# openai/baselines

Measured on NVIDIA H100. Metric: PPO2 learner env-steps/sec, higher is better.
Workload: dtype f16 operands / f32 accumulate (GAE f64 carry)

## Files before the change

baselines_b200/csrc/conv_shift.cu:

```cuda
#include <stdlib.h>

#include <type_traits>

#include "common.cuh"
#include "tc_common.cuh"

namespace b200rl {

static constexpr int SH_BM = 128;
static constexpr int SH_CONSUMER_WARPS = 8;
static constexpr int SH_TMA_WARP = SH_CONSUMER_WARPS;
__host__ __device__ constexpr int sh_threads(bool u8) { return (SH_CONSUMER_WARPS + 1) * 32 + (u8 ? 256 : 0); }
static constexpr int SH_MAX_TAPS = 16;
__host__ __device__ constexpr int sh_arows(int KH) { return KH == 1 ? 160 : 144; }
__host__ __device__ constexpr int sh_stages(int KH) { return KH == 1 ? 6 : 4; }
static constexpr int SH_U8_STAGES = 12;
static constexpr int SH_U8_WRES_BYTES = 16 * 1024;
__host__ __device__ constexpr int sh_wgrad_krows(bool u8) { return u8 ? 128 : 64; }
__host__ __device__ constexpr int sh_wres_bytes(int KH, bool u8) {
  return u8 ? SH_U8_WRES_BYTES : KH == 1 ? 80 * 1024 : 64 * 1024;
}
static constexpr int SH_BAR_BYTES = 512;
__host__ __device__ constexpr int sh_mask_stage_bytes(int BN, bool DACT) { return DACT ? SH_BM * BN / 8 : 0; }
static constexpr int SH_EPI_WARP_BYTES = 16 * 64;
static constexpr int SH_EPI_BYTES = SH_CONSUMER_WARPS * SH_EPI_WARP_BYTES;
static constexpr int SH_WROWS_K = 96;
static constexpr int SH_WABYTES = SH_WROWS_K * 128;
__host__ __device__ constexpr int sh_wgrad_qw(int BN, int KH, bool u8) { return u8 ? 2 : BN == 32 ? 4 : KH == 1 ? 3 : 2; }

static constexpr int SH_ORDER_BAR = 2;
__device__ __forceinline__ void order_wait(int wg) {
  asm volatile("bar.sync %0, %1;" ::"r"(SH_ORDER_BAR + wg), "n"(SH_CONSUMER_WARPS * 32) : "memory");
}
__device__ __forceinline__ void order_pass(int wg) {
  asm volatile("bar.arrive %0, %1;" ::"r"(SH_ORDER_BAR + 1 - wg), "n"(SH_CONSUMER_WARPS * 32) : "memory");
}

struct AddrMap {
  int mode;
  long long sN, sY, sX;
  int Cq, s;
  int Cq_log2, s_log2;
};

__device__ __forceinline__ long long map_rowbase(const AddrMap& a, int n, int y, int x) {
  if (a.mode == 2) {
    const int sm = a.s - 1;
// ... 137 lines not shown
          }
        }
        fence_proxy_async_smem();
        __syncwarp();
        if (lane == 0) {
          if (tile < ntiles) mbar_arrive(&full_bar[s]);
          if (ub == 0) mbar_arrive(&head_bar[s]);
        }
        u8_load(u, row_start, uc + RND, sb[d], lane, q[d]);
        sb[d] = u8_lookup(u, row_start, uc + 2 * RND, total, M, lane);
      }
    }
  }
}

struct ShiftParams {
  U8Src u8;
  FastDiv fwg, fhg;
  long long M;
  int Hg, Wg;
  int N;
  int taps;
  int shift[SH_MAX_TAPS];
  int min_shift;
  int vy, vx;
  __half* out;
  AddrMap omap;
  uint16_t* bits_out;
  const uint16_t* saved_bits;
  const float* bias;
  int act, dact;
  float alpha;
  int num_tiles;
};

__device__ __forceinline__ void stmatrix_x4(uint32_t addr, const uint32_t (&r)[4]) {
  asm volatile("stmatrix.sync.aligned.m8n8.x4.shared.b16 [%0], {%1, %2, %3, %4};" ::"r"(addr), "r"(r[0]), "r"(r[1]),
               "r"(r[2]), "r"(r[3])
               : "memory");
}
__device__ __forceinline__ uint4 ld_shared_v4(uint32_t addr) {
  uint4 v;
  asm volatile("ld.shared.v4.b32 {%0,%1,%2,%3}, [%4];" : "=r"(v.x), "=r"(v.y), "=r"(v.z), "=r"(v.w) : "r"(addr) : "memory");
  return v;
}
__device__ __forceinline__ void st_global_v4(void* p, const uint4& v) {
  asm volatile("st.global.v4.b32 [%0], {%1,%2,%3,%4};" ::"l"(p), "r"(v.x), "r"(v.y), "r"(v.z), "r"(v.w) : "memory");
}
__device__ __forceinline__ uint32_t h2_bits(__half2 h) { return *reinterpret_cast<const uint32_t*>(&h); }
__device__ __forceinline__ uint32_t mask_pair(uint32_t b8, int k) {
  const uint32_t b = b8 >> (2 * k);
  return ((b & 1u) | ((b & 2u) << 15)) * 0xffffu;
}

template <int BN, int KH, bool DACT, bool U8>
__global__ void __launch_bounds__(sh_threads(U8), 1)
conv_shift_fwd_kernel(const __grid_constant__ CUtensorMap tmX, const __grid_constant__ CUtensorMap tmW,
                      const __grid_constant__ ShiftParams p) {
  constexpr int SH_ABYTES = sh_arows(KH) * 128;
  constexpr int STAGE_BYTES = KH * SH_ABYTES;
  constexpr int STAGES = U8 ? SH_U8_STAGES : sh_stages(KH);
  using Ring = U8Ring<SH_BM, STAGES>;
  constexpr bool PINGPONG = !(BN == 128 && !DACT);
  constexpr int MH = PINGPONG ? 2 : 1;
  static_assert(PINGPONG || !U8, "the uint8 ring's release rule assumes ping-pong");
  constexpr int A_PITCH = U8 ? SH_BM * 128 : STAGE_BYTES;
  constexpr int A_TOTAL = U8 ? Ring::BYTES : STAGES * STAGE_BYTES;
  extern __shared__ uint8_t smem_raw[];
  uint8_t* smem = reinterpret_cast<uint8_t*>((reinterpret_cast<uintptr_t>(smem_raw) + 1023) & ~uintptr_t(1023));
  uint8_t* wres = smem + A_TOTAL;
  uint64_t* bars = reinterpret_cast<uint64_t*>(wres + sh_wres_bytes(KH, U8));
  uint64_t* full_bar = bars;
  uint64_t* empty_bar = bars + STAGES;
  uint64_t* w_bar = bars + 2 * STAGES;
  uint64_t* head_bar = bars + 2 * STAGES + 1;
  static_assert((3 * STAGES + 1) * 8 <= SH_BAR_BYTES, "barrier block");
  constexpr int MASK_STAGE = sh_mask_stage_bytes(BN, DACT);
  uint8_t* smask = reinterpret_cast<uint8_t*>(bars) + SH_BAR_BYTES;
  uint8_t* sepi = smask + STAGES * MASK_STAGE;

  __shared__ float s_bias[BN];
  const int warp = threadIdx.x >> 5, lane = threadIdx.x & 31;
  constexpr int w_sub = BN * 128;
  if (threadIdx.x < BN) s_bias[threadIdx.x] = (p.bias && (int)threadIdx.x < p.N) ? p.bias[threadIdx.x] : 0.0f;
  if (threadIdx.x == 0) {
    for (int s = 0; s < STAGES; ++s) {
      mbar_init(&full_bar[s], U8 ? Ring::UPT : 1);
      mbar_init(&empty_bar[s], (U8 || !PINGPONG) ? SH_CONSUMER_WARPS : 4);
      if (U8) mbar_init(&head_bar[s], 1);
    }
    mbar_init(w_bar, 1);
    if (U8)
// ... 11 lines not shown
  } else {
    tile_first = (int)blockIdx.x;
    tile_stride = (int)gridDim.x;
    tile_count = tile_first < p.num_tiles ? (p.num_tiles - tile_first + tile_stride - 1) / tile_stride : 0;
  }

  if (warp == SH_TMA_WARP) {
    if (elect_one()) {
      tma_prefetch_desc(&tmX);
      tma_prefetch_desc(&tmW);
      mbar_arrive_expect_tx(w_bar, (uint32_t)(p.taps * KH) * w_sub);
      for (int q = 0; q < p.taps * KH; ++q) tma_load_2d(wres + q * w_sub, &tmW, w_bar, q * 64, 0);
    }
    __syncwarp();
    int s = 0;
    uint32_t ph = 0;
    if (!U8) {
      for (int i = 0; i < tile_count; ++i) {
        const int tile = tile_first + i * tile_stride;
        mbar_wait(&empty_bar[s], ph ^ 1);
        if (elect_one()) {
          uint8_t* sa = smem + s * STAGE_BYTES;
          uint32_t mbytes = 0;
          const uint8_t* msrc = nullptr;
          if (DACT && p.saved_bits != nullptr) {
            const long long left = p.M - (long long)tile * SH_BM;
            mbytes = (uint32_t)(left < SH_BM ? left : SH_BM) * (BN / 8);
            msrc = reinterpret_cast<const uint8_t*>(p.saved_bits) + (long long)tile * MASK_STAGE;
#pragma unroll 1
            for (uint32_t b = mbytes & ~15u; b < mbytes; b += 4)
              *reinterpret_cast<uint32_t*>(smask + s * MASK_STAGE + b) = __ldg(reinterpret_cast<const uint32_t*>(msrc + b));
            if (mbytes & 15u) __threadfence_block();
          }
          mbar_arrive_expect_tx(&full_bar[s], (uint32_t)STAGE_BYTES + (mbytes & ~15u));
          const int row0 = tile * SH_BM + p.min_shift;
#pragma unroll
          for (int h = 0; h < KH; ++h) tma_load_2d(sa + h * SH_ABYTES, &tmX, &full_bar[s], h * 64, row0);
          if (mbytes >= 16) bulk_load_1d(smask + s * MASK_STAGE, msrc, mbytes & ~15u, &full_bar[s]);
        }
        __syncwarp();
        if (++s == STAGES) { s = 0; ph ^= 1; }
      }
    }
  } else if (U8 && warp > SH_TMA_WARP) {
    u8_ring_producer<SH_BM, STAGES, 2>(p.u8, p.M, (long long)tile_first * SH_BM + p.min_shift, tile_count, smem,
                                       full_bar, head_bar, empty_bar, warp - (SH_TMA_WARP + 1), lane);
  } else {
    const int wg = __shfl_sync(0xffffffffu, warp >> 2, 0), t = threadIdx.x & 127;
    const int row0 = PINGPONG ? 0 : wg * 64;
    const uint32_t w_base = smem_u32(wres);
    const float lo = (p.act == ACT_RELU) ? 0.0f : -INFINITY;
    const __half2 lo2 = __floats2half2_rn(lo, lo);
    const __half2 zero2 = __floats2half2_rn(0.0f, 0.0f);
    const int er = lane & 15, ep = lane >> 4;
    const int erow = row0 + 16 * (warp & 3) + er;
    uint32_t epi_addr[2];
#pragma unroll
    for (int jj = 0; jj < 2; ++jj)
      epi_addr[jj] = smem_u32(sepi + warp * SH_EPI_WARP_BYTES) + er * 64 + (((2 * jj + ep) ^ ((er >> 1) & 3)) << 4);
    const bool masked = DACT && p.saved_bits != nullptr;
    float acc[MH][BN / 2];
    mbar_wait(w_bar, 0);
    for (int i = PINGPONG ? wg : 0; i < tile_count; i += PINGPONG ? 2 : 1) {
      const int tile = tile_first + i * tile_stride;
      const int s = i % STAGES, s1 = (s + 1 == STAGES) ? 0 : s + 1;
      const uint32_t ph = (uint32_t)(i / STAGES) & 1u;
      mbar_wait(&full_bar[s], ph);
      if (U8) mbar_wait(&head_bar[s1], s1 == 0 ? ph ^ 1 : ph);
      if (PINGPONG && i > 0) order_wait(wg);
      const uint32_t a_base = smem_u32(smem + s * A_PITCH) + (uint32_t)(row0 * 128);
      wgmma_fence();
#pragma unroll 1
      for (int a = 0; a < p.taps; ++a) {
        const uint32_t at = a_base + (uint32_t)p.shift[a] * 128u;
        const uint32_t wt = w_base + (uint32_t)(a * KH * w_sub);
#pragma unroll
        for (int h = 0; h < KH; ++h) {
#pragma unroll
          for (int k = 0; k < 4; ++k) {
            const uint64_t bdesc = make_sdesc(wt + h * w_sub + k * 32, 16, 1024, 1);
#pragma unroll
            for (int mh = 0; mh < MH; ++mh) {
              const uint64_t adesc = make_sdesc(at + mh * 64 * 128 + h * SH_ABYTES + k * 32, 16, 1024, 1);
              wgmma_f16<BN, 0, 0>(acc[mh], adesc, bdesc, (a | h | k) ? 1u : 0u);
            }
          }
        }
      }
      wgmma_commit();
      if (PINGPONG && i + 1 < tile_count) order_pass(wg);
      wgmma_wait<0>();
      auto release = [&]() {
        __syncwarp();
        if (lane == 0) {
          mbar_arrive(&empty_bar[s]);
          if (U8) mbar_arrive(&empty_bar[s1]);
        }
      };
      uint32_t mrow[MH][BN / 32];
      if (masked) {
#pragma unroll
        for (int mh = 0; mh < MH; ++mh) {
          const uint32_t r = smem_u32(smask + s * MASK_STAGE) + (uint32_t)((erow + mh * 64) * (BN / 8));
#pragma unroll
          for (int i = 0; i < BN / 32; ++i) asm volatile("ld.shared.b32 %0, [%1];" : "=r"(mrow[mh][i]) : "r"(r + 4 * i));
        }
      } else {
        release();
      }

#pragma unroll
      for (int mh = 0; mh < MH; ++mh) {
        const uint32_t m = (uint32_t)tile * SH_BM + mh * 64 + erow;
        const uint32_t t2 = p.fwg.div(m);
        const int x = (int)(m - t2 * (uint32_t)p.Wg);
        const int n = (int)p.fhg.div(t2);
        const int y = (int)(t2 - (uint32_t)n * (uint32_t)p.Hg);
        const bool ok = ((long long)m < p.M) && (y < p.vy) && (x < p.vx);
        const long long obase = map_rowbase(p.omap, n, y, x);
#pragma unroll
        for (int ps = 0; ps < BN / 32; ++ps) {
#pragma unroll
          for (int jj = 0; jj < 2; ++jj) {
            const int b = 2 * (2 * ps + jj);
            uint32_t r[4];
#pragma unroll
            for (int k = 0; k < 4; ++k) {
              const int e = 4 * (b + (k >> 1)) + 2 * (k & 1);
              const int c = 8 * (b + (k >> 1)) + 2 * (t & 3);
              __half2 o;
              if (DACT) {
                o = __floats2half2_rn(acc[mh][e] * p.alpha, acc[mh][e + 1] * p.alpha);
              } else {
                o = __hmax2(__floats2half2_rn(fmaf(acc[mh][e], p.alpha, s_bias[c]),
                                              fmaf(acc[mh][e + 1], p.alpha, s_bias[c + 1])),
                            lo2);
              }
              r[k] = h2_bits(o);
            }
            stmatrix_x4(epi_addr[jj], r);
          }
          __syncwarp();
#pragma unroll
          for (int jj = 0; jj < 2; ++jj) {
            const int j = 2 * ps + jj;
            uint4 v = ld_shared_v4(epi_addr[jj]);
            const long long ocol = map_coloff(p.omap, 16 * j);
            if (masked) {
              const uint32_t b8 = (mrow[mh][j >> 1] >> (16 * (j & 1) + 8 * ep)) & 0xffu;
              v.x &= mask_pair(b8, 0);
              v.y &= mask_pair(b8, 1);
// ... 224 lines not shown
      }
    }
    if (kb1 > kb0) {
#pragma unroll
      for (int i = 0; i < QW; ++i) {
        if (i < nq) {
#pragma unroll
          for (int e = 0; e < BN / 2; ++e) {
            const int cn = acc_col(t, e);
            const long long grow = (long long)(q0 + i) * 64 + acc_row(t, e);
            if (cn < p.N) p.ws_g[((long long)blockIdx.x * p.grows + grow) * p.N + cn] = acc[i][e] * p.alpha;
          }
        }
      }
    }
  }
  if (ncta > 1) cluster_sync();
}

static U8Src make_u8src(const void* x, const long long* idx, int H, int W, int C, int s) {
  U8Src u{};
  u.x = reinterpret_cast<const uint8_t*>(x);
  if (!x) return u;
  u.idx = idx;
  u.sample_bytes = (long long)H * W * C;
  u.row_bytes = W * C;
  u.y_bytes = s * W * C;
  u.x_bytes = s * C;
  u.per = make_fastdiv((uint32_t)((H / s) * (W / s)));
  u.wg = make_fastdiv((uint32_t)(W / s));
  return u;
}

template <int BN, int KH, bool DACT, bool U8 = false>
static int launch_fwd(const CUtensorMap& tmX, const CUtensorMap& tmW, const ShiftParams& p, cudaStream_t st) {
  constexpr int STAGES = U8 ? SH_U8_STAGES : sh_stages(KH);
  constexpr int SMEM = (U8 ? U8Ring<SH_BM, STAGES>::BYTES : STAGES * KH * sh_arows(KH) * 128) + sh_wres_bytes(KH, U8) +
                       1024 + SH_BAR_BYTES + STAGES * sh_mask_stage_bytes(BN, DACT) + SH_EPI_BYTES;
  static_assert(SMEM + 1024 <= 227 * 1024, "conv_shift_fwd: shared memory budget (+ static bias array)");
  static bool attr = false;
  auto kern = conv_shift_fwd_kernel<BN, KH, DACT, U8>;
  if (!attr) {
    cudaError_t e = cudaFuncSetAttribute(kern, cudaFuncAttributeMaxDynamicSharedMemorySize, SMEM);
    if (e != cudaSuccess) {
      set_last_error("conv_shift_fwd: smem attr %d: %s", SMEM, cudaGetErrorString(e));
      return B200RL_ERR_CUDA;
    }
    attr = true;
  }
  const int grid = p.num_tiles < device_num_sms() ? p.num_tiles : device_num_sms();
  kern<<<grid, sh_threads(U8), SMEM, st>>>(tmX, tmW, p);
  return check_launch("conv_shift_fwd_kernel");
}

static int wgrad_cluster(int groups) {
  int g = groups < 8 ? groups : 8;
  while (groups % g) --g;
  return g;
}

template <int BN, int KH, bool U8 = false>
static int launch_wgrad(const CUtensorMap& tmX, const CUtensorMap& tmD, const ShiftWgradParams& p, dim3 grid,
                        cudaStream_t st) {
  constexpr int STAGES = (KH == 1) ? 8 : 6;
  constexpr int KR = sh_wgrad_krows(U8);
  constexpr int BROWB = (BN >= 64) ? 128 : BN * 2;
  constexpr int B_REGION = (KR * BROWB + 1023) & ~1023;
  constexpr int SMEM =
      (U8 ? U8Ring<KR, STAGES>::BYTES + STAGES * B_REGION : STAGES * (KH * SH_WABYTES + B_REGION)) + 1024 + 512;
  static_assert(SMEM <= 227 * 1024, "conv_shift_wgrad: shared memory budget");
  static bool attr = false;
  static int co_resident[9] = {};
  auto kern = conv_shift_wgrad_kernel<BN, KH, U8>;
  if (!attr) {
// ... 26 lines not shown
        return B200RL_ERR_CUDA;
      }
    }
    if (co_resident[g] * g < device_num_sms()) g = 1;
  }
  cfg.numAttrs = g > 1 ? 1 : 0;
  const cudaError_t e = cudaLaunchKernelEx(&cfg, kern, tmX, tmD, p);
  const int rc = check_launch("conv_shift_wgrad_kernel");
  if (rc == B200RL_OK && e != cudaSuccess) {
    set_last_error("conv_shift_wgrad_kernel: %s", cudaGetErrorString(e));
    return B200RL_ERR_CUDA;
  }
  return rc;
}

static int ilog2(int v) { int l = 0; while ((1 << l) < v) ++l; return l; }
static bool fill_map(AddrMap& a, const long long* m) {
  a.mode = (int)m[0]; a.sN = m[1]; a.sY = m[2]; a.sX = m[3]; a.Cq = (int)m[4]; a.s = (int)m[5];
  a.Cq_log2 = a.s_log2 = 0;
  if (a.mode == 0) return true;
  if (a.Cq < 16 || (a.Cq & (a.Cq - 1)) || a.s < 1 || (a.s & (a.s - 1))) return false;
  a.Cq_log2 = ilog2(a.Cq); a.s_log2 = ilog2(a.s);
  return true;
}

}

using namespace b200rl;

extern "C" int b200rl_conv_shift_fwd(const void* X, long long B, int Hg, int Wg, int C, const void* W, long long ldw,
                                     int N, int taps, const int* shifts, int vy, int vx, void* out,
                                     const long long* omap, const long long* smap, const float* bias, int act, int dact,
                                     float alpha, const void* u8_x, const long long* u8_idx, int u8_H, int u8_W,
                                     int u8_C, int u8_s, void* bits_out, const void* saved_bits, void* stream_) {
  cudaStream_t stream = static_cast<cudaStream_t>(stream_);
  B200RL_REQUIRE((X || u8_x) && W && out && omap && B > 0, "conv_shift_fwd: null operand");
  B200RL_REQUIRE(!(bits_out && dact) && !(saved_bits && !(dact && smap)), "conv_shift_fwd: bits_out is a forward output, saved_bits a dact input (with smap)");
  if (u8_x) {
    B200RL_REQUIRE(C == 64 && u8_s * u8_C == 16 && u8_s == 4 && u8_H == Hg * u8_s && u8_W == Wg * u8_s && !dact &&
                       N == 32 && (reinterpret_cast<uintptr_t>(u8_x) & 15) == 0 && (u8_W * u8_C) % 16 == 0,
                   "conv_shift_fwd: fused uint8 source needs s=4, s*C=16, N=32, 16 B aligned rows");
  }
  B200RL_REQUIRE(C == 64 || C == 128, "conv_shift_fwd: C must be 64 or 128 (got %d)", C);
  B200RL_REQUIRE(N == 32 || N == 64 || N == 128, "conv_shift_fwd: N must be 32, 64 or 128 (got %d)", N);
  B200RL_REQUIRE(taps >= 1 && taps <= SH_MAX_TAPS, "conv_shift_fwd: 1..%d taps", SH_MAX_TAPS);
  B200RL_REQUIRE((C == 64 || C == 128) && (long long)taps * (C / 64) * N * 128 <= sh_wres_bytes(C / 64, u8_x != nullptr),
                 "conv_shift_fwd: weights do not fit in smem");
  ShiftParams p = {};
  int lo = shifts[0], hi = shifts[0];
  for (int t = 1; t < taps; ++t) { lo = shifts[t] < lo ? shifts[t] : lo; hi = shifts[t] > hi ? shifts[t] : hi; }
  B200RL_REQUIRE(hi - lo <= sh_arows(C / 64) - SH_BM, "conv_shift_fwd: shift span %d too large for C = %d", hi - lo,
                 C);
  B200RL_REQUIRE(B * Hg * Wg < (1LL << 31) - 4096, "conv_shift_fwd: too many rows");
  p.M = B * Hg * Wg; p.Hg = Hg; p.Wg = Wg; p.N = N; p.taps = taps; p.min_shift = lo;
  for (int t = 0; t < taps; ++t) p.shift[t] = shifts[t] - lo;
  p.vy = vy; p.vx = vx; p.out = reinterpret_cast<__half*>(out);
  B200RL_REQUIRE(fill_map(p.omap, omap), "conv_shift_fwd: output map needs power-of-two Cq >= 16 and s");
  p.bits_out = reinterpret_cast<uint16_t*>(bits_out);
  p.saved_bits = reinterpret_cast<const uint16_t*>(saved_bits);
  B200RL_REQUIRE(((omap[1] | omap[2] | omap[3]) & 15) == 0 && (reinterpret_cast<uintptr_t>(out) & 31) == 0,
                 "conv_shift_fwd: output strides must be multiples of 16 elements, base 32-byte aligned");
  if (saved_bits)
    B200RL_REQUIRE(smap[0] == 0 && smap[3] == N && smap[2] == (long long)Wg * N && smap[1] == (long long)Hg * Wg * N &&
                       (reinterpret_cast<uintptr_t>(saved_bits) & 15) == 0,
                   "conv_shift_fwd: saved_bits needs the row-contiguous map (0, Hg*Wg*N, Wg*N, N) and a 16-byte aligned "
                   "base");
  p.bias = bias; p.act = act; p.dact = dact; p.alpha = alpha;
  p.num_tiles = (int)((p.M + SH_BM - 1) / SH_BM);
  p.u8 = make_u8src(u8_x, u8_idx, u8_H, u8_W, u8_C, u8_s);
  B200RL_REQUIRE(Hg >= 2 && Wg >= 2, "conv_shift_fwd: grid must be at least 2x2");
  p.fwg = make_fastdiv((uint32_t)Wg);
  p.fhg = make_fastdiv((uint32_t)Hg);
  CUtensorMap tmX, tmW;
  int rc;
  B200RL_REQUIRE(act == ACT_NONE || act == ACT_RELU, "conv_shift_fwd: activation must be none or relu");
  if ((rc = make_tmap_2d_f16(&tmW, W, N, (long long)taps * C, ldw, 64, N)) != 0) return rc;
  if (u8_x) {
    B200RL_REQUIRE(hi - lo <= 32, "conv_shift_fwd: uint8-fed shift span %d exceeds one 32-row unit", hi - lo);
    return launch_fwd<32, 1, false, true>(tmW, tmW, p, stream);
  }
  if ((rc = make_tmap_2d_f16(&tmX, X, p.M, C, C, 64, sh_arows(C / 64))) != 0) return rc;
  const int KH = C / 64;
#define SHIFT_FWD_CASE(bn)                                                                                    \
  if (N == bn) {                                                                                              \
    if (dact) return KH == 1 ? launch_fwd<bn, 1, true>(tmX, tmW, p, stream) : launch_fwd<bn, 2, true>(tmX, tmW, p, stream); \
    return KH == 1 ? launch_fwd<bn, 1, false>(tmX, tmW, p, stream) : launch_fwd<bn, 2, false>(tmX, tmW, p, stream);        \
  }
  SHIFT_FWD_CASE(32)
  SHIFT_FWD_CASE(64)
  SHIFT_FWD_CASE(128)
#undef SHIFT_FWD_CASE
  return B200RL_ERR_UNSUPPORTED;
}

extern "C" int b200rl_conv_shift_wgrad(const void* X, long long rows, int C, const void* dY, int N, int taps,
                                       const int* shifts, float* G, long long ldg, float alpha, float* gbias,
                                       float alpha_b, int max_ctas, const void* u8_x, const long long* u8_idx, int u8_H,
                                       int u8_W, int u8_C, int u8_s, int kx, void* stream_) {
  cudaStream_t stream = static_cast<cudaStream_t>(stream_);
  B200RL_REQUIRE((X || u8_x) && dY && G && rows > 0, "conv_shift_wgrad: null operand");
  if (kx < 1) kx = 1;
  B200RL_REQUIRE(kx <= 3, "conv_shift_wgrad: kx must be 1..3");
  if (u8_x)
    B200RL_REQUIRE(C == 64 && u8_s == 4 && u8_s * u8_C == 16 && N == 32 && u8_H % 4 == 0 && u8_W % 4 == 0 &&
                       (reinterpret_cast<uintptr_t>(u8_x) & 15) == 0,
                   "conv_shift_wgrad: fused uint8 source needs s=4, s*C=16, N=32");
  B200RL_REQUIRE(C == 64 || C == 128, "conv_shift_wgrad: C must be 64 or 128");
  B200RL_REQUIRE(N == 32 || N == 64, "conv_shift_wgrad: N must be 32 or 64 (got %d)", N);
  B200RL_REQUIRE(taps >= 1 && taps <= SH_MAX_TAPS, "conv_shift_wgrad: 1..%d taps", SH_MAX_TAPS);
  const int KH = C / 64;
  ShiftWgradParams p = {};
  for (int t = 0; t < taps; ++t) {
    B200RL_REQUIRE(shifts[t] >= 0 && shifts[t] + kx - 1 <= SH_WROWS_K - 64, "conv_shift_wgrad: shift %d out of range",
// ... 35 lines not shown
```

baselines_b200/nn.py:

```python
import functools
import math
from collections import OrderedDict, namedtuple

import numpy as np
import torch

from . import ops

NATURE_CONVS = (("c1", 32, 8, 4), ("c2", 64, 4, 2), ("c3", 64, 3, 1))


def _pad8(n):
    return (n + 7) // 8 * 8


def ortho_init(shape, scale, rng=np.random):
    shape = tuple(shape)
    flat = shape if len(shape) == 2 else (int(np.prod(shape[:-1])), shape[-1])
    a = rng.normal(0.0, 1.0, flat)
    u, _, v = np.linalg.svd(a, full_matrices=False)
    q = (u if u.shape == flat else v).reshape(shape)
    return (scale * q[:shape[0], :shape[1]]).astype(np.float32)


# ... 306 lines not shown
    def cast_jobs(self):
        return self.wx.cast_jobs() + [ops.CastJob(self.wh, self.H, 4 * self.H, self.wh16, 4 * self.H, self.whT16, self.H,
                                                  1.0)]

    def refresh(self):
        for j in self.cast_jobs():
            ops.cast_transpose(*j)

    def forward(self, x, ldx, seq, train=True):
        H, rows = self.H, seq.T * seq.B
        self.wx.forward(x, ldx, rows, self.xg, 4 * H, mode=ops.MODE_F32_STORE, act=ops.ACT_NONE)
        ops.lstm_seq_fwd(self.xg, 4 * H, self.wh16, seq.masks, seq.state, self.h, H, seq.T, seq.B, H,
                         mask_idx=seq.mask_idx, state_idx=seq.state_idx, state_out=seq.state_out,
                         hprev_out=self.hprev if train else None, gates_out=self.xg if train else None,
                         c_out=self.c if train else None)
        self._x, self._ldx, self._seq = x, ldx, seq
        return self.h, H

    def backward(self, alpha, dx=None, ldo=0, saved=None, ld_saved=0, act=ops.ACT_NONE):
        H, seq = self.H, self._seq
        rows = seq.T * seq.B
        ops.lstm_seq_bwd(self.dh, H, self.xg, self.c, seq.masks, seq.state, self.whT16, self.dz, 4 * H, seq.T, seq.B, H,
                         mask_idx=seq.mask_idx, state_idx=seq.state_idx)
        tiles = -(-H // 128) * -(-4 * H // 256)
        kb = -(-rows // 64)
        split = max(1, min(kb // 2 if kb >= 2 else 1, -(-2 * ops.num_sms() // tiles)))
        ops.gemm(self.hprev, self.dz, self.gwh, M=H, N=4 * H, K=rows, lda=H, ldb=4 * H, ldc=4 * H, mn_major=True,
                 mode=ops.MODE_F32_ATOMIC, alpha=alpha, split_k=split, tag="wgrad.lstm/wh")
        self.wx.wgrad(self._x, self._ldx, self.dz, 4 * H, rows, alpha)
        if dx is not None:
            self.wx.dgrad(self.dz, 4 * H, rows, dx, ldo, saved=saved, ld_saved=ld_saved, act=act)


ConvLayerPlan = namedtuple("ConvLayerPlan", "path s2d geom implicit_dgrad kx")
ConvLayerPlan.__doc__ = """How one conv layer runs.  path: "shift" (csrc/conv_shift.cu), "implicit" (TMA im2col GEMM over the
input viewed as geom = (H, W, C, R, S, stride_h, stride_w, pad_t, pad_l)) or "explicit" (im2col + GEMM).  s2d: the
layer reads its input space-to-depth'ed (and its master weight rows are stored in that order).  implicit_dgrad: the
data gradient is one implicit GEMM with the pixel-shuffle epilogue instead of GEMM + col2im.  kx: taps per filter row
the shift-GEMM weight gradient folds into one pass."""
ConvStackPlan = namedtuple("ConvStackPlan", "shift fused_u8 layers")
ConvStackPlan.__doc__ = """shift: every layer runs as shift-GEMM, and every layer writes its 1-bit ReLU mask, which the next
data gradient (or fc1's) reads.  fused_u8: the first shift layer reads the uint8 frames itself."""

_XFOLD_WGRAD = ((2, 32, 64), (2, 64, 64), (2, 64, 128), (3, 64, 64))


def _shift_stack_ok(ob_shape, convs):
    H, W, C = ob_shape
    for i, (_nm, nf, rf, st) in enumerate(convs):
        if rf % st or H % st or W % st:
            return False
        k, Hg, Wg, Cg = rf // st, H // st, W // st, C * st * st
        span = (k - 1) * Wg + (k - 1)
        if Cg not in (64, 128) or k * k > 16 or Hg < 2 or Wg < 2 or nf not in (32, 64):
            return False
        if span > (32 if Cg == 64 else 16) or k * k * (Cg // 64) * nf * 128 > (80 if Cg == 64 else 64) * 1024:
            return False
        if i > 0 and nf != 64:
            return False
        OH, OW = ops._conv_out(H, W, rf, st, False)
        if i + 1 < len(convs):
            nrf, nst = convs[i + 1][2], convs[i + 1][3]
            if OH % nst or OW % nst:
                return False
            kn = nrf // nst
            if nf * nst * nst not in (64, 128) or kn * kn * nf * nst * nst * 128 > 80 * 1024:
                return False
        H, W, C = OH, OW, nf
    return True


def _implicit_geom(H, W, C, rf, st, same_pad, s2d):
    if s2d:
        return (H // st, W // st, C * st * st, rf // st, rf // st, 1, 1, 0, 0)
    pad_t = pad_l = 0
    if same_pad:
        OH, OW = ops._conv_out(H, W, rf, st, True)
        pad_t, pad_l = max((OH - 1) * st + rf - H, 0) // 2, max((OW - 1) * st + rf - W, 0) // 2
    m = 64 // C if C in (16, 32) else 1
    if m > 1 and W % m == 0 and rf % m == 0 and st % m == 0 and pad_l % m == 0:
        return (H, W // m, C * m, rf, rf // m, st, st // m, pad_t, pad_l // m)
    if C in (16, 32, 64):
        return (H, W, C, rf, rf, st, st, pad_t, pad_l)
    if 16 % C == 0 and (W * C) % 16 == 0 and (rf * C) % 16 == 0 and (st * C) % 16 == 0 and (pad_l * C) % 16 == 0:
        k = 16 // C
        return (H, W // k, 16, rf, rf // k, st, st // k, pad_t, pad_l // k)
    return None


def plan_conv_stack(ob_shape, convs, same_pad, has_fc):
    if not same_pad and _shift_stack_ok(ob_shape, convs):
        if not has_fc:
            raise NotImplementedError("shift-mode conv_only towers")
        H, W, C = ob_shape
        layers = []
        for _nm, nf, rf, st in convs:
            k, Cg = rf // st, C * st * st
            OH, OW = ops._conv_out(H, W, rf, st, False)
            assert (OH * OW * nf) % 16 == 0
            layers.append(ConvLayerPlan("shift", st > 1, None, False, k if (k, nf, Cg) in _XFOLD_WGRAD else 1))
            H, W, C = OH, OW, nf
        _nm, nf0, rf0, st0 = convs[0]
        fused_u8 = st0 == 4 and ob_shape[2] == 4 and nf0 == 32 and (rf0 // st0) ** 2 * nf0 * 128 <= 16 * 1024
        return ConvStackPlan(True, fused_u8, layers)
    H, W, C = ob_shape
    layers = []
    for i, (_nm, nf, rf, st) in enumerate(convs):
        s2d = (i == 0 and st > 1 and not same_pad and rf % st == 0 and H % st == 0 and W % st == 0 and
               C * st * st in (16, 32, 64) and (st * C) % 8 == 0 and (W * C) % 8 == 0)
        geom = _implicit_geom(H, W, C, rf, st, same_pad, s2d)
        implicit_dgrad = i > 0 and geom is not None and not same_pad and nf in (16, 32, 64) and C % 16 == 0
        layers.append(ConvLayerPlan("explicit" if geom is None else "implicit", s2d, geom, implicit_dgrad, 1))
        H, W = ops._conv_out(H, W, rf, st, same_pad)
        C = nf
    return ConvStackPlan(False, False, layers)


class Tower:

    def __init__(self, store, kind, ob_shape, prefix, tf_prefix, rng, cap, init="ortho", num_layers=2,
                 num_hidden=64, convs=NATURE_CONVS, same_pad=False, fc_hidden=512, tf_style="a2c", onehot_n=0,
                 onehot_nvec=None, nlstm=128, layer_norm=False):
        if layer_norm and kind != "mlp":
            raise NotImplementedError("layer_norm is an argument of 'mlp' (common/models.py:75); layer-normalised LSTMs "
                                      "(lnlstm, cnn_lnlstm) are not implemented")
        self.kind, self.cap, self.store = kind, cap, store
        self.base = {"lstm": "mlp", "cnn_lstm": "cnn"}.get(kind, kind)
        if kind == "lstm":
            num_layers = 0
        self.convs, self.fcs = [], []
        self.lns = []
        self.lstm = None
        winit = (lambda shape, scale: ortho_init(shape, scale, rng)) if init == "ortho" else \
                (lambda shape, scale: xavier_uniform(shape, rng))
        if self.base in ("cnn", "conv_only"):
            H, W, C = ob_shape
            self.in_u8 = True
            scale_in = 1.0 / 255.0
            self.plan = plan_conv_stack(ob_shape, convs, same_pad, self.base == "cnn")
            self.shift_mode = self.plan.shift
            for i, ((nm, nf, rf, stride), lp) in enumerate(zip(convs, self.plan.layers)):
                if tf_style == "a2c":
                    tfw, tfb, bshape = f"{tf_prefix}/{nm}/w:0", f"{tf_prefix}/{nm}/b:0", (1, nf, 1, 1)
                else:
                    cn = "Conv" if i == 0 else f"Conv_{i}"
# ... 57 lines not shown
        if self.convs and self.shift_mode:
            self._materialize_shift(f16)
            self.hfc = [torch.empty(cap, l.Np, **f16) for l in self.fcs]
            self.dzfc = [torch.empty(cap, l.Np, **f16) for l in self.fcs]
            self.ld_hfc = [l.Np for l in self.fcs]
            self.dlatent, self.ld_dlatent = self.dzfc[-1], self.fcs[-1].Np
            return
        self.cols = [None if c.implicit else torch.empty(cap * c.P, c.K, **f16) for c in self.convs]
        self.hconv = [torch.empty(cap * c.P, c.nf, **f16) for c in self.convs]
        self.dcols = [None] + [None if c.implicit_dgrad else torch.empty(cap * c.P, c.K, **f16)
                               for c in self.convs[1:]]
        self.dzconv = [torch.zeros(cap * c.P, c.nf, **f16) for c in self.convs]
        if self.convs and self.convs[0].implicit and self.in_u8:
            c0 = self.convs[0]
            self.x16 = torch.empty(cap, c0.H * c0.W * c0.C, **f16)
        self.hfc = [torch.empty(cap, l.Np, **f16) for l in self.fcs]
        self.dzfc = [torch.empty(cap, l.Np, **f16) for l in self.fcs]
        self.ld_hfc = [l.Np for l in self.fcs]
        if self.base == "mlp":
            self.x0 = torch.zeros(cap, 2 * self.in_pad, **f16)
            self.obs_overflow = torch.zeros(1, dtype=torch.int32, device=dev)
            self.ob_seg = ops.segment_table(self.onehot_nvec, dev) if self.onehot_nvec else None
        if self.fcs:
            self.dlatent, self.ld_dlatent = self.dzfc[-1], self.fcs[-1].Np
        elif self.convs:
            self.dlatent, self.ld_dlatent = self.dzconv[-1], self.flat

    def _materialize_shift(self, f16):
        cap, cv = self.cap, self.convs
        self.sg = []
        for c, lp in zip(cv, self.plan.layers):
            s_, k = c.stride, c.rf // c.stride
            Hg, Wg, Cg = c.H // s_, c.W // s_, c.C * s_ * s_
            self.sg.append(dict(Hg=Hg, Wg=Wg, Cg=Cg, k=k, s=s_, kx=lp.kx,
                                shifts=[a * Wg + b for a in range(k) for b in range(k)],
                                yshifts=[a * Wg for a in range(k)]))
        g0 = self.sg[0]
        self.fused_u8 = self.plan.fused_u8
        self.x16 = None if self.fused_u8 else torch.empty(cap, g0["Hg"] * g0["Wg"] * g0["Cg"], **f16)
        self.hconv = [torch.empty(cap, c.OH * c.OW * c.nf, **f16) for c in cv]
        self.hbits = [torch.zeros(cap * (c.OH * c.OW * c.nf // 16), dtype=torch.int16, device=self.hconv[i].device)
                      for i, c in enumerate(cv)]
        self.dY = [torch.zeros(cap, g["Hg"] * g["Wg"] * c.nf, **f16) for c, g in zip(cv, self.sg)]
        self.wd = [None] + [torch.zeros(g["Cg"], g["k"] * g["k"] * c.nf, **f16) for c, g in zip(cv[1:], self.sg[1:])]
        self.flat = cv[-1].OH * cv[-1].OW * cv[-1].nf

    def _forward_shift(self, x, B, src_idx, masks=True):
        cv, sg = self.convs, self.sg
        c0 = cv[0]
        if self.fused_u8:
            self._u8 = (x, src_idx, c0.H, c0.W, c0.C, c0.stride)
            cur = None
        else:
            self._u8 = None
            ops.s2d_gather(x, self.x16, B, c0.H, c0.W, c0.C, c0.stride, src_idx=src_idx)
            cur = self.x16
        for i, (c, g) in enumerate(zip(cv, sg)):
            if i + 1 < len(cv) and cv[i + 1].stride > 1:
                sn = cv[i + 1].stride
                Hn, Wn, Cn = c.OH // sn, c.OW // sn, c.nf * sn * sn
                omap = (2, Hn * Wn * Cn, Wn * Cn, Cn, c.nf, sn)
            else:
                omap = (0, c.OH * c.OW * c.nf, c.OW * c.nf, c.nf, 0, 0)
            ops.conv_shift_fwd(cur, B, g["Hg"], g["Wg"], g["Cg"], c.w_fwd, c.Kp, c.nf, g["shifts"], c.OH, c.OW,
                               self.hconv[i], omap, bias=c.b, act=c.act, tag="fwd." + c.name,
                               u8=self._u8 if i == 0 else None, bits_out=self.hbits[i] if masks else None,
                               useful_rows=B * c.OH * c.OW)
            cur = self.hconv[i]
        return cur, self.flat

    def _backward_shift(self, B, alpha):
        cv, sg = self.convs, self.sg
        for i in reversed(range(len(cv))):
            c, g = cv[i], sg[i]
            rows = B * g["Hg"] * g["Wg"]
            xin = self.x16 if i == 0 else self.hconv[i - 1]
            ops.conv_shift_wgrad(xin, rows, g["Cg"], self.dY[i], c.nf, g["yshifts"] if g["kx"] > 1 else g["shifts"],
                                 c.gw, c.nf, alpha=alpha * c.in_scale, tag="wgrad." + c.name, gbias=c.gb,
                                 alpha_b=alpha, u8=self._u8 if i == 0 else None, useful_rows=B * c.OH * c.OW,
                                 kx=g["kx"])
            if i == 0:
                break
            cp, gp = cv[i - 1], sg[i - 1]
            omap = (1, gp["Hg"] * gp["Wg"] * cp.nf, gp["Wg"] * cp.nf, cp.nf, cp.nf, g["s"])
            smap = (0, g["Hg"] * g["Wg"] * g["Cg"], g["Wg"] * g["Cg"], g["Cg"], 0, 0)
            ops.conv_shift_fwd(self.dY[i], B, g["Hg"], g["Wg"], c.nf, self.wd[i], g["k"] * g["k"] * c.nf, g["Cg"],
                               [-sft for sft in g["shifts"]], g["Hg"], g["Wg"], self.dY[i - 1], omap,
                               smap=smap, act=ops.ACT_RELU, dact=True, tag="dgrad." + c.name,
                               saved_bits=self.hbits[i - 1], useful_rows=B * c.OH * c.OW)

    def cast_jobs(self):
        jobs = [j for l in self.layers for j in l.cast_jobs()]
        if self.convs and self.shift_mode:
            for c, g, wd in zip(self.convs[1:], self.sg[1:], self.wd[1:]):
                taps, Cg, nf = g["k"] * g["k"], g["Cg"], c.nf
                jobs += [ops.CastJob(c.w[t * Cg:(t + 1) * Cg], Cg, nf, wd[:, t * nf:], taps * nf, None, 0, 1.0)
                         for t in range(taps)]
        if self.lstm is not None:
            jobs += self.lstm.cast_jobs()
        return jobs
# ... 158 lines not shown
```

baselines_b200/ops.py:

```python
from collections import namedtuple

import torch

from . import _lib

MODE_F16_ACT, MODE_F32_STORE, MODE_F32_ATOMIC, MODE_F16_DACT, MODE_F16_SHUFFLE = 0, 1, 2, 3, 4
ACT_NONE, ACT_RELU, ACT_TANH = 0, 1, 2
ACT_CODES = {None: ACT_NONE, "none": ACT_NONE, "relu": ACT_RELU, "tanh": ACT_TANH}


def _ptr(t):
    return None if t is None else t.data_ptr()


def _stream():
    return torch.cuda.current_stream().cuda_stream


_SMS = {}


def num_sms():
    d = torch.cuda.current_device()
    if d not in _SMS:
# ... 40 lines not shown


def conv_gemm(x, B, H, W, C, R, S, stride_h, stride_w, pad_h, pad_w, OH, OW, wt_or_dz, ldb, out, ldc, N, kind,
              mode, act=ACT_NONE, alpha=1.0, bias=None, saved=None, ld_saved=0, split_k=1, shuffle=None, tag=None):
    _chk(x, torch.float16, "x")
    _chk(wt_or_dz, torch.float16, "wt_or_dz")
    sh = shuffle or (0, 0, 0, 0)
    rows = B * OH * OW
    _lib.call("b200rl_conv_gemm", _ptr(x), int(B), H, W, C, R, S, stride_h, stride_w, pad_h, pad_w, OH, OW,
              _ptr(wt_or_dz), int(ldb), _ptr(out), int(ldc), _ptr(bias), _ptr(saved), int(ld_saved), int(N), int(kind),
              int(mode), int(act), float(alpha), int(split_k), int(sh[0]), int(sh[1]), int(sh[2]), int(sh[3]),
              _stream(), label="conv." + (tag or str(kind)), flops=2.0 * rows * N * R * S * C,
              nbytes=2.0 * B * H * W * C + 2.0 * R * S * C * N + rows * N * (2.0 if kind == 0 else 2.0))


import ctypes as _C


def _iarr(vals, ctype):
    return (ctype * len(vals))(*[int(v) for v in vals])


def _u8_args(u8):
    if u8 is None:
        return None, None, 0, 0, 0, 0
    x, idx, H, W, C, s = u8
    _chk(x, torch.uint8, "u8 images")
    _chk(idx, torch.int64, "u8 src_idx")
    return _ptr(x), _ptr(idx), int(H), int(W), int(C), int(s)


def conv_shift_fwd(X, B, Hg, Wg, C, W, ldw, N, shifts, vy, vx, out, omap, *, smap=None, bias=None,
                   act=ACT_NONE, dact=False, alpha=1.0, tag=None, u8=None, bits_out=None, saved_bits=None,
                   useful_rows=None):
    _chk(X, torch.float16, "X")
    _chk(W, torch.float16, "W")
    _chk(out, torch.float16, "out")
    u8a = _u8_args(u8)
    _chk(bits_out, torch.int16, "bits_out")
    _chk(saved_bits, torch.int16, "saved_bits")
    sh = _iarr(shifts, _C.c_int)
    om = _iarr(omap, _C.c_longlong)
    sm = _iarr(smap, _C.c_longlong) if smap is not None else None
    rows = B * Hg * Wg
    useful = float(useful_rows) if useful_rows is not None else float(B) * vy * vx
    if dact:
        nbytes = 2.0 * useful * C + 2.0 * rows * N
        nbytes += 0.0 if saved_bits is None else 0.125 * rows * N
    else:
        nbytes = (1.0 if u8 is not None else 2.0) * rows * C + 2.0 * useful * N + (0.125 * useful * N if bits_out is not None else 0.0)
    _lib.call("b200rl_conv_shift_fwd", _ptr(X), int(B), Hg, Wg, C, _ptr(W), int(ldw), int(N), len(shifts), sh, vy, vx,
              _ptr(out), om, sm, _ptr(bias), int(act), int(bool(dact)), float(alpha), *u8a,
              _ptr(bits_out), _ptr(saved_bits), _stream(),
              label="convs." + (tag or "fwd"), flops=2.0 * useful * N * len(shifts) * C, nbytes=nbytes)


def conv_shift_wgrad(X, rows, C, dY, N, shifts, G, ldg, alpha=1.0, max_ctas=0, tag=None, gbias=None, alpha_b=1.0,
                     u8=None, useful_rows=None, kx=1):
    _chk(X, torch.float16, "X")
    _chk(dY, torch.float16, "dY")
    _chk(G, torch.float32, "G")
    sh = _iarr(shifts, _C.c_int)
    _chk(gbias, torch.float32, "gbias")
    u8a = _u8_args(u8)
    _lib.call("b200rl_conv_shift_wgrad", _ptr(X), int(rows), C, _ptr(dY), int(N), len(shifts), sh, _ptr(G), int(ldg),
              float(alpha), _ptr(gbias), float(alpha_b), int(max_ctas), *u8a, int(kx), _stream(),
              label="convs." + (tag or "wgrad"),
              flops=2.0 * (float(useful_rows) if useful_rows is not None else rows) * N * len(shifts) * kx * C,
              nbytes=rows * (1.0 if u8 is not None else 2.0) * C +
              2.0 * N * (float(useful_rows) if useful_rows is not None else rows))


def dgrad_weights(w, out, R, S, Cin, Cout, s, ld):
    _chk(w, torch.float32, "w")
    _chk(out, torch.float16, "out")
    _lib.call("b200rl_dgrad_weights", _ptr(w), _ptr(out), R, S, Cin, Cout, s, int(ld), _stream())


def _conv_out(H, W, rf, stride, same_pad):
    if same_pad:
        return -(-H // stride), -(-W // stride)
    return (H - rf) // stride + 1, (W - rf) // stride + 1


def im2col(x, cols, B, H, W, C, rf, stride, same_pad=False, src_idx=None, tag=None):
    _chk(src_idx, torch.int64, "src_idx")
# ... 414 lines not shown
```

include/b200rl.h:

```cpp
#ifndef B200RL_H
#define B200RL_H
#include <stdint.h>
#ifdef __cplusplus
extern "C" {
#endif

#define B200RL_OK 0
#define B200RL_ERR_ARG (-1)
#define B200RL_ERR_CUDA (-2)
#define B200RL_ERR_UNSUPPORTED (-3)
#define B200RL_ERR_DRIVER (-4)

#define B200RL_MODE_F16_ACT 0
#define B200RL_MODE_F32_STORE 1
#define B200RL_MODE_F32_ATOMIC 2
#define B200RL_MODE_F16_DACT 3
#define B200RL_MODE_F16_SHUFFLE 4
#define B200RL_ACT_NONE 0
#define B200RL_ACT_RELU 1
#define B200RL_ACT_TANH 2

const char* b200rl_last_error(void);
int b200rl_version(void);

int b200rl_gae_scan(const float* rewards, const float* values, const uint8_t* dones, const float* last_values,
                    const uint8_t* last_dones, float* advs, float* returns, int T, int N, double gamma, double lam,
                    int variant, void* stream);

int b200rl_gemm_f16(const void* A, const void* B, void* C, const float* bias, const void* saved, int M, int N, int K,
                    long long lda, long long ldb, long long ldc, long long ld_saved, int mn_major, int mode, int act,
                    float alpha, int split_k, int max_ctas, int rm_C, int rm_OW, int rm_Wg, const void* saved_bits,
                    void* stream);

int b200rl_conv_shift_fwd(const void* X, long long B, int Hg, int Wg, int C, const void* W, long long ldw, int N,
                          int taps, const int* shifts, int vy, int vx, void* out, const long long* omap,
                          const long long* smap, const float* bias, int act, int dact, float alpha,
                          const void* u8_x, const long long* u8_idx, int u8_H, int u8_W, int u8_C, int u8_s,
                          void* act_bits_out, const void* saved_bits, void* stream);
int b200rl_conv_shift_wgrad(const void* X, long long rows, int C, const void* dY, int N, int taps, const int* shifts,
                            float* G, long long ldg, float alpha, float* gbias, float alpha_b, int max_ctas,
                            const void* u8_x, const long long* u8_idx, int u8_H, int u8_W, int u8_C, int u8_s,
                            int kx, void* stream);

int b200rl_conv_gemm(const void* x, long long B, int H, int W, int C, int R, int S, int stride_h, int stride_w,
                     int pad_h, int pad_w, int OH, int OW, const void* Wt_or_dz, long long ldb, void* out,
                     long long ldc, const float* bias, const void* saved, long long ld_saved, int N, int kind,
                     int mode, int act, float alpha, int split_k, int sh_H, int sh_W, int sh_C, int sh_s,
                     void* stream);
int b200rl_dgrad_weights(const float* w, void* out, int R, int S, int Cin, int Cout, int s, long long ld,
                         void* stream);

int b200rl_im2col(const void* x, int src_is_u8, const long long* src_idx, void* cols, long long B, int H, int W,
                  int C, int rf, int stride, int same_pad, void* stream);
int b200rl_frame_stack(const void* prev, const void* frame, const void* news, void* out, long long N, long long pixels,
                       int nstack, int c, void* stream);

int b200rl_s2d_gather(const void* x, const long long* src_idx, void* out, long long B, int H, int W, int C, int s,
                      void* stream);
int b200rl_col2im(const void* dcols, const void* saved, void* dx, long long B, int H, int W, int C, int rf,
                  int stride, int same_pad, int act, void* stream);
int b200rl_colsum(const void* dz, float* db, long long rows, int C, long long ld, float alpha, void* stream);

int b200rl_cat_step(const float* logits, long long ld, int nA, const int* seg_off, int nseg, const float* vpred,
                    long long ldv, const float* uniforms, unsigned long long seed, unsigned long long offset,
                    const unsigned long long* offset_dev, long long* actions, float* values, float* neglogp,
                    long long B, void* stream);
int b200rl_bern_step(const float* logits, long long ld, int n, const float* vpred, long long ldv,
                     const float* uniforms, unsigned long long seed, unsigned long long offset,
                     const unsigned long long* offset_dev, float* actions, float* values, float* neglogp, long long B,
                     void* stream);
int b200rl_gauss_step(const float* mean, long long ld, const float* logstd, int d, const float* vpred,
// ... 98 lines not shown
```

Baseline: 1.209 million.

## Add sample-tiled shift-GEMM forward that skips dead grid rows per sample

Adds a sample-tiled mode to the shift-conv forward kernel. Each 128-row tile covers two samples, 64 output rows each, loaded via per-sample TMA boxes of 88 rows. This skips output grid rows that are only computed and discarded in the flat row tiling. The planner enables it for 64-channel layers whose valid outputs fit in the first 64 rows of a sample. In exchange it adds per-sample TMA loads and a new template variant, and the gain depends on the share of dead rows.

```diff
diff --git a/baselines_b200/csrc/conv_shift.cu b/baselines_b200/csrc/conv_shift.cu
--- a/baselines_b200/csrc/conv_shift.cu
+++ b/baselines_b200/csrc/conv_shift.cu
@@ -12,7 +12,9 @@
 static constexpr int SH_TMA_WARP = SH_CONSUMER_WARPS;
 __host__ __device__ constexpr int sh_threads(bool u8) { return (SH_CONSUMER_WARPS + 1) * 32 + (u8 ? 256 : 0); }
 static constexpr int SH_MAX_TAPS = 16;
-__host__ __device__ constexpr int sh_arows(int KH) { return KH == 1 ? 160 : 144; }
+static constexpr int SH_ST_ROWS = 64;
+static constexpr int SH_ST_AROWS = 88;
+__host__ __device__ constexpr int sh_arows(int KH, bool ST = false) { return ST ? 2 * SH_ST_AROWS : KH == 1 ? 160 : 144; }
 __host__ __device__ constexpr int sh_stages(int KH) { return KH == 1 ? 6 : 4; }
 static constexpr int SH_U8_STAGES = 12;
 static constexpr int SH_U8_WRES_BYTES = 16 * 1024;
@@ -216,6 +218,7 @@
   int act, dact;
   float alpha;
   int num_tiles;
+  int B;
 };
 
 __device__ __forceinline__ void stmatrix_x4(uint32_t addr, const uint32_t (&r)[4]) {
@@ -237,11 +240,13 @@
   return ((b & 1u) | ((b & 2u) << 15)) * 0xffffu;
 }
 
-template <int BN, int KH, bool DACT, bool U8>
+template <int BN, int KH, bool DACT, bool U8, bool ST = false>
 __global__ void __launch_bounds__(sh_threads(U8), 1)
 conv_shift_fwd_kernel(const __grid_constant__ CUtensorMap tmX, const __grid_constant__ CUtensorMap tmW,
                       const __grid_constant__ ShiftParams p) {
-  constexpr int SH_ABYTES = sh_arows(KH) * 128;
+  static_assert(!ST || (KH == 1 && !DACT && !U8), "sample tiling: TMA-fed 64-channel forward only");
+  constexpr int SH_ABYTES = sh_arows(KH, ST) * 128;
+  constexpr int MH_PITCH = (ST ? SH_ST_AROWS : 64) * 128;
   constexpr int STAGE_BYTES = KH * SH_ABYTES;
   constexpr int STAGES = U8 ? SH_U8_STAGES : sh_stages(KH);
   using Ring = U8Ring<SH_BM, STAGES>;
@@ -319,10 +324,18 @@
               *reinterpret_cast<uint32_t*>(smask + s * MASK_STAGE + b) = __ldg(reinterpret_cast<const uint32_t*>(msrc + b));
             if (mbytes & 15u) __threadfence_block();
           }
-          mbar_arrive_expect_tx(&full_bar[s], (uint32_t)STAGE_BYTES + (mbytes & ~15u));
-          const int row0 = tile * SH_BM + p.min_shift;
-#pragma unroll
-          for (int h = 0; h < KH; ++h) tma_load_2d(sa + h * SH_ABYTES, &tmX, &full_bar[s], h * 64, row0);
+          if (ST) {
+            const int n0 = 2 * tile, nb = (n0 + 1 < p.B) ? 2 : 1;
+            const int P = p.Hg * p.Wg;
+            mbar_arrive_expect_tx(&full_bar[s], (uint32_t)(nb * SH_ST_AROWS * 128));
+            for (int b = 0; b < nb; ++b)
+              tma_load_2d(sa + b * MH_PITCH, &tmX, &full_bar[s], 0, (n0 + b) * P + p.min_shift);
+          } else {
+            mbar_arrive_expect_tx(&full_bar[s], (uint32_t)STAGE_BYTES + (mbytes & ~15u));
+            const int row0 = tile * SH_BM + p.min_shift;
+#pragma unroll
+            for (int h = 0; h < KH; ++h) tma_load_2d(sa + h * SH_ABYTES, &tmX, &full_bar[s], h * 64, row0);
+          }
           if (mbytes >= 16) bulk_load_1d(smask + s * MASK_STAGE, msrc, mbytes & ~15u, &full_bar[s]);
         }
         __syncwarp();
@@ -368,7 +381,7 @@
             const uint64_t bdesc = make_sdesc(wt + h * w_sub + k * 32, 16, 1024, 1);
 #pragma unroll
             for (int mh = 0; mh < MH; ++mh) {
-              const uint64_t adesc = make_sdesc(at + mh * 64 * 128 + h * SH_ABYTES + k * 32, 16, 1024, 1);
+              const uint64_t adesc = make_sdesc(at + mh * MH_PITCH + h * SH_ABYTES + k * 32, 16, 1024, 1);
               wgmma_f16<BN, 0, 0>(acc[mh], adesc, bdesc, (a | h | k) ? 1u : 0u);
             }
           }
@@ -398,12 +411,21 @@
 
 #pragma unroll
       for (int mh = 0; mh < MH; ++mh) {
-        const uint32_t m = (uint32_t)tile * SH_BM + mh * 64 + erow;
-        const uint32_t t2 = p.fwg.div(m);
-        const int x = (int)(m - t2 * (uint32_t)p.Wg);
-        const int n = (int)p.fhg.div(t2);
-        const int y = (int)(t2 - (uint32_t)n * (uint32_t)p.Hg);
-        const bool ok = ((long long)m < p.M) && (y < p.vy) && (x < p.vx);
+        int n, y, x;
+        bool ok;
+        if (ST) {
+          n = 2 * tile + mh;
+          y = (int)p.fwg.div((uint32_t)erow);
+          x = erow - y * p.Wg;
+          ok = (n < p.B) && (y < p.vy) && (x < p.vx);
+        } else {
+          const uint32_t m = (uint32_t)tile * SH_BM + mh * 64 + erow;
+          const uint32_t t2 = p.fwg.div(m);
+          x = (int)(m - t2 * (uint32_t)p.Wg);
+          n = (int)p.fhg.div(t2);
+          y = (int)(t2 - (uint32_t)n * (uint32_t)p.Hg);
+          ok = ((long long)m < p.M) && (y < p.vy) && (x < p.vx);
+        }
         const long long obase = map_rowbase(p.omap, n, y, x);
 #pragma unroll
         for (int ps = 0; ps < BN / 32; ++ps) {
@@ -694,14 +716,15 @@
   return u;
 }
 
-template <int BN, int KH, bool DACT, bool U8 = false>
+template <int BN, int KH, bool DACT, bool U8 = false, bool ST = false>
 static int launch_fwd(const CUtensorMap& tmX, const CUtensorMap& tmW, const ShiftParams& p, cudaStream_t st) {
   constexpr int STAGES = U8 ? SH_U8_STAGES : sh_stages(KH);
-  constexpr int SMEM = (U8 ? U8Ring<SH_BM, STAGES>::BYTES : STAGES * KH * sh_arows(KH) * 128) + sh_wres_bytes(KH, U8) +
-                       1024 + SH_BAR_BYTES + STAGES * sh_mask_stage_bytes(BN, DACT) + SH_EPI_BYTES;
+  constexpr int SMEM = (U8 ? U8Ring<SH_BM, STAGES>::BYTES : STAGES * KH * sh_arows(KH, ST) * 128) +
+                       sh_wres_bytes(KH, U8) + 1024 + SH_BAR_BYTES + STAGES * sh_mask_stage_bytes(BN, DACT) +
+                       SH_EPI_BYTES;
   static_assert(SMEM + 1024 <= 227 * 1024, "conv_shift_fwd: shared memory budget (+ static bias array)");
   static bool attr = false;
-  auto kern = conv_shift_fwd_kernel<BN, KH, DACT, U8>;
+  auto kern = conv_shift_fwd_kernel<BN, KH, DACT, U8, ST>;
   if (!attr) {
     cudaError_t e = cudaFuncSetAttribute(kern, cudaFuncAttributeMaxDynamicSharedMemorySize, SMEM);
     if (e != cudaSuccess) {
@@ -794,11 +817,13 @@
                                      int N, int taps, const int* shifts, int vy, int vx, void* out,
                                      const long long* omap, const long long* smap, const float* bias, int act, int dact,
                                      float alpha, const void* u8_x, const long long* u8_idx, int u8_H, int u8_W,
-                                     int u8_C, int u8_s, void* bits_out, const void* saved_bits, void* stream_) {
+                                     int u8_C, int u8_s, void* bits_out, const void* saved_bits, int sample_tiled,
+                                     void* stream_) {
   cudaStream_t stream = static_cast<cudaStream_t>(stream_);
   B200RL_REQUIRE((X || u8_x) && W && out && omap && B > 0, "conv_shift_fwd: null operand");
   B200RL_REQUIRE(!(bits_out && dact) && !(saved_bits && !(dact && smap)), "conv_shift_fwd: bits_out is a forward output, saved_bits a dact input (with smap)");
   if (u8_x) {
+    B200RL_REQUIRE(!sample_tiled, "conv_shift_fwd: the fused uint8 source is not sample-tiled");
     B200RL_REQUIRE(C == 64 && u8_s * u8_C == 16 && u8_s == 4 && u8_H == Hg * u8_s && u8_W == Wg * u8_s && !dact &&
                        N == 32 && (reinterpret_cast<uintptr_t>(u8_x) & 15) == 0 && (u8_W * u8_C) % 16 == 0,
                    "conv_shift_fwd: fused uint8 source needs s=4, s*C=16, N=32, 16 B aligned rows");
@@ -841,6 +866,16 @@
     B200RL_REQUIRE(hi - lo <= 32, "conv_shift_fwd: uint8-fed shift span %d exceeds one 32-row unit", hi - lo);
     return launch_fwd<32, 1, false, true>(tmW, tmW, p, stream);
   }
+  if (sample_tiled) {
+    B200RL_REQUIRE(!dact && C == 64 && N == 64, "conv_shift_fwd: sample tiling is a forward with C = N = 64");
+    B200RL_REQUIRE((vy - 1) * Wg + vx <= SH_ST_ROWS && hi - lo <= SH_ST_AROWS - SH_ST_ROWS,
+                   "conv_shift_fwd: sample tiling needs valid outputs in the first %d rows of a sample and a shift "
+                   "span <= %d", SH_ST_ROWS, SH_ST_AROWS - SH_ST_ROWS);
+    p.B = (int)B;
+    p.num_tiles = (int)((B + 1) / 2);
+    if ((rc = make_tmap_2d_f16(&tmX, X, p.M, C, C, 64, SH_ST_AROWS)) != 0) return rc;
+    return launch_fwd<64, 1, false, false, true>(tmX, tmW, p, stream);
+  }
   if ((rc = make_tmap_2d_f16(&tmX, X, p.M, C, C, 64, sh_arows(C / 64))) != 0) return rc;
   const int KH = C / 64;
 #define SHIFT_FWD_CASE(bn)                                                                                    \
diff --git a/baselines_b200/nn.py b/baselines_b200/nn.py
--- a/baselines_b200/nn.py
+++ b/baselines_b200/nn.py
@@ -362,12 +362,13 @@
             self.wx.dgrad(self.dz, 4 * H, rows, dx, ldo, saved=saved, ld_saved=ld_saved, act=act)
 
 
-ConvLayerPlan = namedtuple("ConvLayerPlan", "path s2d geom implicit_dgrad kx")
+ConvLayerPlan = namedtuple("ConvLayerPlan", "path s2d geom implicit_dgrad kx sample_tiled")
 ConvLayerPlan.__doc__ = """How one conv layer runs.  path: "shift" (csrc/conv_shift.cu), "implicit" (TMA im2col GEMM over the
 input viewed as geom = (H, W, C, R, S, stride_h, stride_w, pad_t, pad_l)) or "explicit" (im2col + GEMM).  s2d: the
 layer reads its input space-to-depth'ed (and its master weight rows are stored in that order).  implicit_dgrad: the
 data gradient is one implicit GEMM with the pixel-shuffle epilogue instead of GEMM + col2im.  kx: taps per filter row
-the shift-GEMM weight gradient folds into one pass."""
+the shift-GEMM weight gradient folds into one pass.  sample_tiled: the shift-GEMM forward works one sample per 64-row
+block and skips the sample's dead grid rows (_sample_tiled)."""
 ConvStackPlan = namedtuple("ConvStackPlan", "shift fused_u8 layers")
 ConvStackPlan.__doc__ = """shift: every layer runs as shift-GEMM, and every layer writes its 1-bit ReLU mask, which the next
 data gradient (or fc1's) reads.  fused_u8: the first shift layer reads the uint8 frames itself."""
@@ -400,6 +401,11 @@
     return True
 
 
+def _sample_tiled(Hg, Wg, Cg, k, OH, OW, nf, u8):
+    return (not u8 and Cg == 64 and nf == 64 and Hg * Wg > 64 and (OH - 1) * Wg + OW <= 64 and
+            (k - 1) * Wg + (k - 1) <= 24)
+
+
 def _implicit_geom(H, W, C, rf, st, same_pad, s2d):
     if s2d:
         return (H // st, W // st, C * st * st, rf // st, rf // st, 1, 1, 0, 0)
@@ -422,16 +428,17 @@
     if not same_pad and _shift_stack_ok(ob_shape, convs):
         if not has_fc:
             raise NotImplementedError("shift-mode conv_only towers")
+        _nm, nf0, rf0, st0 = convs[0]
+        fused_u8 = st0 == 4 and ob_shape[2] == 4 and nf0 == 32 and (rf0 // st0) ** 2 * nf0 * 128 <= 16 * 1024
         H, W, C = ob_shape
         layers = []
-        for _nm, nf, rf, st in convs:
+        for i, (_nm, nf, rf, st) in enumerate(convs):
             k, Cg = rf // st, C * st * st
             OH, OW = ops._conv_out(H, W, rf, st, False)
             assert (OH * OW * nf) % 16 == 0
-            layers.append(ConvLayerPlan("shift", st > 1, None, False, k if (k, nf, Cg) in _XFOLD_WGRAD else 1))
+            tiled = _sample_tiled(H // st, W // st, Cg, k, OH, OW, nf, fused_u8 and i == 0)
+            layers.append(ConvLayerPlan("shift", st > 1, None, False, k if (k, nf, Cg) in _XFOLD_WGRAD else 1, tiled))
             H, W, C = OH, OW, nf
-        _nm, nf0, rf0, st0 = convs[0]
-        fused_u8 = st0 == 4 and ob_shape[2] == 4 and nf0 == 32 and (rf0 // st0) ** 2 * nf0 * 128 <= 16 * 1024
         return ConvStackPlan(True, fused_u8, layers)
     H, W, C = ob_shape
     layers = []
@@ -440,7 +447,7 @@
                C * st * st in (16, 32, 64) and (st * C) % 8 == 0 and (W * C) % 8 == 0)
         geom = _implicit_geom(H, W, C, rf, st, same_pad, s2d)
         implicit_dgrad = i > 0 and geom is not None and not same_pad and nf in (16, 32, 64) and C % 16 == 0
-        layers.append(ConvLayerPlan("explicit" if geom is None else "implicit", s2d, geom, implicit_dgrad, 1))
+        layers.append(ConvLayerPlan("explicit" if geom is None else "implicit", s2d, geom, implicit_dgrad, 1, False))
         H, W = ops._conv_out(H, W, rf, st, same_pad)
         C = nf
     return ConvStackPlan(False, False, layers)
@@ -564,7 +571,7 @@
         for c, lp in zip(cv, self.plan.layers):
             s_, k = c.stride, c.rf // c.stride
             Hg, Wg, Cg = c.H // s_, c.W // s_, c.C * s_ * s_
-            self.sg.append(dict(Hg=Hg, Wg=Wg, Cg=Cg, k=k, s=s_, kx=lp.kx,
+            self.sg.append(dict(Hg=Hg, Wg=Wg, Cg=Cg, k=k, s=s_, kx=lp.kx, tiled=lp.sample_tiled,
                                 shifts=[a * Wg + b for a in range(k) for b in range(k)],
                                 yshifts=[a * Wg for a in range(k)]))
         g0 = self.sg[0]
@@ -597,7 +604,7 @@
             ops.conv_shift_fwd(cur, B, g["Hg"], g["Wg"], g["Cg"], c.w_fwd, c.Kp, c.nf, g["shifts"], c.OH, c.OW,
                                self.hconv[i], omap, bias=c.b, act=c.act, tag="fwd." + c.name,
                                u8=self._u8 if i == 0 else None, bits_out=self.hbits[i] if masks else None,
-                               useful_rows=B * c.OH * c.OW)
+                               useful_rows=B * c.OH * c.OW, sample_tiled=g["tiled"])
             cur = self.hconv[i]
         return cur, self.flat
 
diff --git a/baselines_b200/ops.py b/baselines_b200/ops.py
--- a/baselines_b200/ops.py
+++ b/baselines_b200/ops.py
@@ -96,7 +96,7 @@
 
 def conv_shift_fwd(X, B, Hg, Wg, C, W, ldw, N, shifts, vy, vx, out, omap, *, smap=None, bias=None,
                    act=ACT_NONE, dact=False, alpha=1.0, tag=None, u8=None, bits_out=None, saved_bits=None,
-                   useful_rows=None):
+                   useful_rows=None, sample_tiled=False):
     _chk(X, torch.float16, "X")
     _chk(W, torch.float16, "W")
     _chk(out, torch.float16, "out")
@@ -115,7 +115,7 @@
         nbytes = (1.0 if u8 is not None else 2.0) * rows * C + 2.0 * useful * N + (0.125 * useful * N if bits_out is not None else 0.0)
     _lib.call("b200rl_conv_shift_fwd", _ptr(X), int(B), Hg, Wg, C, _ptr(W), int(ldw), int(N), len(shifts), sh, vy, vx,
               _ptr(out), om, sm, _ptr(bias), int(act), int(bool(dact)), float(alpha), *u8a,
-              _ptr(bits_out), _ptr(saved_bits), _stream(),
+              _ptr(bits_out), _ptr(saved_bits), int(bool(sample_tiled)), _stream(),
               label="convs." + (tag or "fwd"), flops=2.0 * useful * N * len(shifts) * C, nbytes=nbytes)
 
 
diff --git a/include/b200rl.h b/include/b200rl.h
--- a/include/b200rl.h
+++ b/include/b200rl.h
@@ -36,7 +36,7 @@
                           int taps, const int* shifts, int vy, int vx, void* out, const long long* omap,
                           const long long* smap, const float* bias, int act, int dact, float alpha,
                           const void* u8_x, const long long* u8_idx, int u8_H, int u8_W, int u8_C, int u8_s,
-                          void* act_bits_out, const void* saved_bits, void* stream);
+                          void* act_bits_out, const void* saved_bits, int sample_tiled, void* stream);
 int b200rl_conv_shift_wgrad(const void* X, long long rows, int C, const void* dY, int N, int taps, const int* shifts,
                             float* G, long long ldg, float alpha, float* gbias, float alpha_b, int max_ctas,
                             const void* u8_x, const long long* u8_idx, int u8_H, int u8_W, int u8_C, int u8_s,
```

After: 1.224 million, median of 6. 1.01x the previous value.
